# HuajianUP/Photo-SLAM

Hardware: AMD Instinct MI355X
Metric: train iters/s (render + L1/SSIM loss + backward + Adam), 2M Gaussians @1080p (higher is better)
Workload: dtype f32; 1 GPU; C3: Replica room0 @1080p shape; gaussians=2000000, width=1920, height=1080, sh_degree=3, parallelism=single GPU, raster_only=False, densify_interval=0, cull_empty_tiles=False, binning=depth-first, sh_adam_fused_into_backward=True, sh_adam_lazy_window=32, scene_index_order=random, geometry_adam_fused_into_backward=True, gaussians_after=2000000

## Files before the change

include/gsr.h:

```cpp
#ifndef GSR_H
#define GSR_H
#include <stddef.h>
#include <stdint.h>
#ifdef __cplusplus
extern "C" {
#endif

typedef enum gsr_status {
	GSR_OK = 0,
	GSR_ERR_INVALID_ARG = -1,
	GSR_ERR_ALLOC = -2,
	GSR_ERR_HIP = -3,
	GSR_ERR_UNSUPPORTED = -4
} gsr_status;

typedef char* (*gsr_alloc_fn)(void* ctx, size_t bytes);

#define GSR_SH_LAZY_WINDOW 32
typedef struct gsr_sh_adam_lazy {
	int* row_step;
	int window;
	double lr_past[GSR_SH_LAZY_WINDOW];
	double lr_tail_past[GSR_SH_LAZY_WINDOW];
} gsr_sh_adam_lazy;
// ... 120 lines not shown
	int packed_capacity_rows;
	const float* dL_ddepth;
	const float* dL_dalpha;
	float* dL_dviewmatrix;
	float* dL_dprojmatrix;
	float* dL_dcampos;
	char* pose_scratch;
	const gsr_geom_reg* geom_reg;
} gsr_backward_args;

int gsr_backward(const gsr_backward_args* args, void* stream);

int gsr_sh_adam_flush(int P, const gsr_sh_adam* adam, void* stream);

int gsr_sh_grad_from_views(int P, int D, int M, int n_views, const float* means3D, const float* campos,
                           long long campos_stride, const float* dL_dcolor_views, long long view_stride, float scale,
                           float* dL_dsh, void* stream);

int gsr_sh_adam_from_views(int P, int D, int M, int n_views, const float* means3D, const float* campos,
                           long long campos_stride, const float* dL_dcolor_views, long long view_stride, float scale,
                           float* shs, const gsr_sh_adam* sh_adam, void* stream);
size_t gsr_packed_view_words(int P, int capacity_rows);
int gsr_pack_view_plan(int P, const int* radii, uint32_t* message, void* scratch, void* stream);
size_t gsr_pack_scratch_bytes(int P);
int gsr_pack_color_view(int P, const float* dL_dcolor_view, const float* campos, int capacity_rows, uint32_t* message, void* scratch,
                        void* stream);
int gsr_sh_grad_from_packed_views(int P, int D, int M, int n_views, const float* means3D, const uint32_t* messages,
                                  long long msg_stride, float scale, float* dL_dsh, void* stream);
int gsr_sh_adam_from_packed_views(int P, int D, int M, int n_views, const float* means3D, const uint32_t* messages,
                                  long long msg_stride, float scale, float* shs, const gsr_sh_adam* sh_adam, void* stream);
int gsr_last_visible_count(void);
int gsr_last_forward_only(void);
long long gsr_depth_resort_count(void);
int gsr_binning_tile_first(int raw_params, int P, int width, int height);
int gsr_check_packed_views(int P, int n_views, const uint32_t* messages, long long msg_stride, int capacity_rows, void* stream);
int gsr_host_wait_stats(double* total_us, long long* calls, int reset);

int gsr_sh_adam_lazy_slice(int P, const gsr_sh_adam* adam, int ahead, void* stream);

int gsr_mark_visible(int P, const float* means3D, const float* viewmatrix, const float* projmatrix,
                     uint8_t* present, void* stream);

int gsr_knn_mean_dist2(int P, const float* points, float* meanDists,
                       gsr_alloc_fn scratchBuffer, void* scratch_ctx, void* stream);

size_t gsr_loss_scratch_bytes(int width, int height);
int gsr_l1_ssim_loss(const float* rendered, const float* gt, const float* mask, int width, int height,
                     float lambda_dssim, float* grad_rendered, float* loss, char* scratch, void* stream);

size_t gsr_loss_exposure_scratch_bytes(int width, int height);
int gsr_l1_ssim_loss_exposure(const float* rendered, const float* gt, const float* mask, int width, int height,
                              float lambda_dssim, const float* exposure, float* grad_rendered, float* grad_exposure,
                              float* loss, char* scratch, void* stream);
int gsr_apply_exposure(const float* image, const float* exposure, int width, int height, float* out, void* stream);

size_t gsr_depth_loss_scratch_bytes(int width, int height);
int gsr_depth_l1_loss(const float* depth, const float* gt_depth, int width, int height, float min_depth, float max_depth,
                      float weight, float* grad_depth, float* loss, char* scratch, void* stream);

int gsr_adam_step(float* param, const float* grad, float* exp_avg, float* exp_avg_sq, long long n, double lr,
                  double beta1, double beta2, double eps, int step, int period, int split, double lr_tail, void* stream);

typedef struct gsr_adam_multi_tensor {
	float* param;
	const float* grad;
	float* exp_avg;
// ... 77 lines not shown
```

photo-slam_amd/capi.py:

```python
import ctypes as C
import os

_HERE = os.path.dirname(os.path.abspath(__file__))
HIP_LIB_PATH = os.path.join(_HERE, "libgsr_hip.so")

ALLOC_FN = C.CFUNCTYPE(C.c_void_p, C.c_void_p, C.c_size_t)

GSR_OK = 0


class GsrError(RuntimeError):
    def __init__(self, lib, status, where):
        msg = lib.gsr_strerror(status).decode()
        hip = lib.gsr_last_hip_error_string().decode()
        super().__init__(f"{where}: {msg} (status {status})" + (f" [{hip}]" if status == -3 and hip else ""))
        self.status = status


class ForwardArgs(C.Structure):
    _fields_ = [("P", C.c_int), ("D", C.c_int), ("M", C.c_int), ("background", C.c_void_p),
                ("width", C.c_int), ("height", C.c_int), ("means3D", C.c_void_p), ("shs", C.c_void_p),
                ("colors_precomp", C.c_void_p), ("opacities", C.c_void_p), ("scales", C.c_void_p),
                ("scale_modifier", C.c_float), ("rotations", C.c_void_p), ("cov3D_precomp", C.c_void_p),
                ("viewmatrix", C.c_void_p), ("projmatrix", C.c_void_p), ("cam_pos", C.c_void_p),
# ... 79 lines not shown
                ("packed_view", C.c_void_p), ("packed_capacity_rows", C.c_int),
                ("dL_ddepth", C.c_void_p), ("dL_dalpha", C.c_void_p),
                ("dL_dviewmatrix", C.c_void_p), ("dL_dprojmatrix", C.c_void_p), ("dL_dcampos", C.c_void_p),
                ("pose_scratch", C.c_void_p), ("geom_reg", C.POINTER(GeomReg))]

class DensifySelectArgs(C.Structure):
    _fields_ = [("P", C.c_int), ("xyz_gradient_accum", C.c_void_p), ("denom", C.c_void_p), ("scaling", C.c_void_p),
                ("opacity", C.c_void_p), ("percent_dense", C.c_float), ("max_grad", C.c_float), ("min_opacity", C.c_float),
                ("extent", C.c_float), ("max_screen_size", C.c_int), ("prune_mask", C.c_void_p)]


class DensifyGatherArgs(C.Structure):
    _fields_ = [("P", C.c_int), ("n_new", C.c_int), ("n_keep", C.c_int), ("n_clone", C.c_int), ("n_child", C.c_int),
                ("n_split", C.c_int), ("features_row_floats", C.c_int),
                ("param_in", C.c_void_p * 5), ("exp_avg_in", C.c_void_p * 5), ("exp_avg_sq_in", C.c_void_p * 5),
                ("param_out", C.c_void_p * 5), ("exp_avg_out", C.c_void_p * 5), ("exp_avg_sq_out", C.c_void_p * 5),
                ("samples", C.c_void_p), ("stats_out", C.c_void_p * 3), ("exist_since_iter_in", C.c_void_p),
                ("exist_since_iter_out", C.c_void_p), ("morton_scratch", C.c_void_p)]


RAW_OPACITY, RAW_SCALING, RAW_ROTATION = 1, 2, 4
CULL_EMPTY_TILES, FORWARD_ONLY = 8, 128
ANTIALIAS = 256
CONTRIBUTION = 512


EXPORTED_SYMBOLS = [
    "gsr_forward", "gsr_backward", "gsr_mark_visible", "gsr_knn_mean_dist2", "gsr_geometry_bytes", "gsr_binning_bytes",
    "gsr_image_bytes", "gsr_knn_scratch_bytes", "gsr_sh_grad_from_views", "gsr_sh_adam_from_views", "gsr_sh_adam_flush", "gsr_sh_adam_lazy_slice", "gsr_adam_step_multi", "gsr_strerror", "gsr_last_hip_error", "gsr_last_hip_error_string",
    "gsr_backend", "gsr_profile_enable", "gsr_profile_stage_count", "gsr_profile_stage_name", "gsr_profile_read",
    "gsr_loss_scratch_bytes", "gsr_l1_ssim_loss", "gsr_adam_step", "gsr_densify_stats", "gsr_densify_scratch_bytes",
    "gsr_densify_select", "gsr_densify_gather", "gsr_transform_points", "gsr_scale_transform_points", "gsr_reproject_depth_pinhole",
    "gsr_neighborhood_depth_pinhole", "gsr_packed_view_words", "gsr_pack_scratch_bytes", "gsr_pack_color_view", "gsr_pack_view_plan",
    "gsr_sh_grad_from_packed_views", "gsr_sh_adam_from_packed_views", "gsr_last_visible_count", "gsr_check_packed_views", "gsr_depth_resort_count",
    "gsr_host_wait_stats", "gsr_binning_tile_first", "gsr_densify_morton_scratch_bytes",
    "gsr_binning_bytes_for", "gsr_image_bytes_for", "gsr_last_forward_only",
    "gsr_depth_loss_scratch_bytes", "gsr_depth_l1_loss", "gsr_pose_grad_scratch_bytes",
    "gsr_loss_exposure_scratch_bytes", "gsr_l1_ssim_loss_exposure", "gsr_apply_exposure",
    "gsr_geom_reg_scratch_bytes",
]

_libs = {}


def load(path=None):
    path = os.path.abspath(path or HIP_LIB_PATH)
    if path in _libs:
        return _libs[path]
    if not os.path.exists(path):
        raise FileNotFoundError(
            f"{path} not found: build the HIP extension first (python photo-slam_amd/build.py or "
            f"__graft_entry__.build()); there is no CPU fallback.")
    L = C.CDLL(path)
    vp, sz, i32, f32 = C.c_void_p, C.c_size_t, C.c_int, C.c_float
    L.gsr_forward.restype = i32
    L.gsr_forward.argtypes = [C.POINTER(ForwardArgs), ALLOC_FN, vp, ALLOC_FN, vp, ALLOC_FN, vp, vp, C.POINTER(i32)]
    L.gsr_backward.restype = i32
    L.gsr_backward.argtypes = [C.POINTER(BackwardArgs), vp]
    L.gsr_sh_grad_from_views.restype = i32
    L.gsr_sh_grad_from_views.argtypes = [i32, i32, i32, i32, vp, vp, C.c_longlong, vp, C.c_longlong, f32, vp, vp]
    L.gsr_sh_adam_from_views.restype = i32
    L.gsr_sh_adam_from_views.argtypes = [i32, i32, i32, i32, vp, vp, C.c_longlong, vp, C.c_longlong, f32, vp, C.POINTER(ShAdam), vp]
    L.gsr_sh_adam_flush.restype = i32
    L.gsr_sh_adam_flush.argtypes = [i32, C.POINTER(ShAdam), vp]
    L.gsr_sh_adam_lazy_slice.restype = i32
    L.gsr_sh_adam_lazy_slice.argtypes = [i32, C.POINTER(ShAdam), i32, vp]
    L.gsr_adam_step_multi.restype = i32
# ... 88 lines not shown
```

photo-slam_amd/csrc/gsr_api.hip:

```cpp
#include <atomic>
#include <chrono>
#include <cmath>
#include <vector>
#include "kernels.h"
#include "shrows.h"

#include <stdio.h>
#include <stdlib.h>
#include <string.h>

namespace gsr {

static thread_local int t_last_err = 0;
static thread_local char t_last_what[256] = {0};
void set_last_hip_error(int err, const char* what)
{
	t_last_err = err;
	snprintf(t_last_what, sizeof(t_last_what), "%s: %s", what ? what : "?", hipGetErrorString((hipError_t)err));
}

struct HostSync {
	uint32_t* pinned = nullptr;
	uint32_t* pinned_dev = nullptr;
	hipEvent_t ev = nullptr;
// ... 82 lines not shown
static bool lazy_slice_early(const gsr_sh_adam* o)
{
	static const int env = env_int("GSR_LAZY_SLICE_EARLY", -1);
	return env >= 0 ? env != 0 : !(o && o->lazy_slice_late);
}
static bool cov3D_stored()
{
	static const int env = env_int("GSR_COV3D_STORED", 0);
	return env != 0;
}
static bool emit_seeded()
{
	static const int env = env_int("GSR_EMIT_SEEDS", 1);
	return env != 0;
}
static int xcd_deal_mode(int tiles)
{
	static const int env = env_int("GSR_XCD_CHUNK", -1);
	if (env >= 0) return env;
	int c = 8;
	while (c > 1 && tiles < 8 * 16 * c) c >>= 1;
	return c;
}
static bool blend_bwd_half_tiles(int tiles)
{
	const char* e = getenv("GSR_BWD_HALF_TILES");
	if (e && *e) {
		static bool logged = false;
		if (!logged) fprintf(stderr, "[gsr] environment override GSR_BWD_HALF_TILES=%s\n", e);
		logged = true;
		return atoi(e) != 0;
	}
	return tiles >= 24 * 256;
}
static int depth_sort_wide()
{
	static const int on = env_int("GSR_DEPTH_SORT_9BIT", 1);
	static const int bits = env_int("GSR_DEPTH_SORT_BITS", 3 * RADIX_BITS_WIDE);
	if (!on) return 0;
	return (bits >= 1 && bits <= 27 && (div_up(bits, RADIX_BITS_WIDE) & 1)) ? bits : 3 * RADIX_BITS_WIDE;
}
static thread_local long long t_depth_resorts = 0;
static bool emit_hist()
{
	static const int env = env_int("GSR_EMIT_HIST", 1);
	return env != 0;
}
constexpr int TILE_FIRST_MAX_GAUSSIANS = 256 * 1024;
static bool binning_tile_first(int raw_params, int P, int tiles)
{
	static const int env = env_int("GSR_BINNING", -1);
	if (env >= 0) return env != 0;
	if (raw_params & GSR_BINNING_TILE_FIRST) return true;
	if (raw_params & GSR_BINNING_DEPTH_FIRST) return false;
	(void)tiles;
	return P <= TILE_FIRST_MAX_GAUSSIANS;
}
static int side_blocks(const gsr_sh_adam* o)
{
	static const int env = env_int("GSR_SH_ADAM_SIDE_BLOCKS", -1);
	return env >= 0 ? env : (o && o->side_blocks > 0 ? o->side_blocks : 256);
}

enum { ST_PREPROCESS = 0, ST_DEPTH_SORT, ST_OFFSET_SCAN, ST_EMIT, ST_TILE_SORT, ST_TILE_RANGES, ST_TILE_DEPTH_SORT, ST_BLEND_FWD,
       ST_GRAD_MEMSET, ST_BLEND_BWD, ST_PREPROCESS_BWD, ST_COUNT };
constexpr int ST_FWD_COUNT = ST_BLEND_FWD + 1;
// ... 424 lines not shown
	if (lazy && slice_early && (st = launch_lazy_slice()) != GSR_OK) return fail(st);
	PROF_BWD(0);
	if (R > 0 && !rows_path) GSR_HIP(hipMemsetAsync(bs.touched, 0, touched_clear_bytes((size_t)R), stream));
	PROF_BWD(1);
	if (R > 0) {
		BlendBwdParams bp;
		bp.ranges = im.ranges; bp.point_list = point_list; bp.rec = g.rec; bp.bg = a->background;
		bp.final_T = im.final_T; bp.n_contrib = im.n_contrib; bp.dL_dpix = a->dL_dpix;
		bp.partials = bs.partials;
		bp.touched = bs.touched;
		bp.contrib = bs.contrib; bp.contrib_stride = (size_t)R;
		bp.W = W; bp.H = H; bp.grid_x = grid_x; bp.tiles = tiles;
		bp.deal = make_tile_deal(tiles, grid_x, xcd_deal_mode(tiles));
		bp.half_tiles = blend_bwd_half_tiles(tiles) ? 1 : 0;
		bp.depth = reinterpret_cast<const float*>(g.depth_key);
		bp.dL_ddepth = a->dL_ddepth; bp.dL_dalpha = a->dL_dalpha;
		if ((st = launch_blend_bwd(bp, stream)) != GSR_OK) return fail(st);
	}
	PROF_BWD(2);
	if (lazy && !slice_early && (st = launch_lazy_slice()) != GSR_OK) return fail(st);

	PreprocessBwdParams pb;
	pb.P = P; pb.D = a->D; pb.M = a->M;
	pb.means3D = a->means3D; pb.radii = a->radii ? a->radii : g.radii; pb.shs = a->shs; pb.clamped = g.clamped;
	pb.scales = a->scales; pb.rotations = a->rotations; pb.scale_modifier = a->scale_modifier;
	pb.cov3D = a->cov3D_precomp;
	if (!pb.cov3D && cov3D_stored()) pb.cov3D = g.cov3D;
	pb.view = a->viewmatrix; pb.proj = a->projmatrix; pb.campos = a->campos;
	pb.focal_y = H / (2.0f * a->tan_fovy);
	pb.focal_x = W / (2.0f * a->tan_fovx);
	pb.tan_fovx = a->tan_fovx; pb.tan_fovy = a->tan_fovy;
	pb.tiles_touched = g.tiles_touched; pb.partials = R > 0 ? bs.partials : nullptr; pb.touched = R > 0 ? bs.touched : nullptr;
	pb.long_runs = g.long_runs; pb.long_counts = g.long_counts; pb.long_capacity = g.long_capacity;
	pb.half_w = 0.5f * (float)W; pb.half_h = 0.5f * (float)H;
	pb.rec = g.rec; pb.raw_params = a->raw_params;
	pb.dL_dmean2D = a->dL_dmean2D; pb.dL_dconic = a->dL_dconic; pb.dL_dopacity = a->dL_dopacity; pb.dL_dcolor = a->dL_dcolor;
	pb.dL_dmean3D = a->dL_dmean3D; pb.dL_dcov3D = a->dL_dcov3D; pb.dL_dsh = a->dL_dsh; pb.dL_dscale = a->dL_dscale;
	pb.dL_drot = a->dL_drot;
	pb.dL_dcolor_view = a->dL_dcolor_view;
	pb.packed_msg = a->dL_dcolor_view ? a->packed_view : nullptr;
	pb.packed_capacity = a->packed_capacity_rows;
	pb.stat_accum = a->stat_grad_accum; pb.stat_denom = a->stat_denom; pb.stat_max_radii = a->stat_max_radii;
	pb.adam_param = nullptr; pb.adam_exp_avg = nullptr; pb.adam_exp_avg_sq = nullptr;
	pb.adam = AdamScalars{};
	pb.adam_skip_culled = 0;
	pb.lazy_row_step = nullptr; pb.lazy_step = 0;
	pb.touched_clear = (R > 0 && rows_path) ? bs.touched : nullptr;
	pb.touched_clear_bytes = (uint32_t)touched_clear_bytes((size_t)R);
	if (a->sh_adam && !pre_slice) {
		const gsr_sh_adam& o = *a->sh_adam;
		pb.adam_param = o.param;
		pb.adam_exp_avg = o.exp_avg; pb.adam_exp_avg_sq = o.exp_avg_sq;
		pb.adam = adam_scalars(o.lr, o.lr_tail, o.beta1, o.beta2, o.eps, o.step);
		pb.adam_skip_culled = (side_busy || lazy) ? 1 : 0;
		if (lazy) { pb.lazy_row_step = la.row_step; pb.lazy_step = la.step; }
	}
	pb.geom = geom;
	pb.depth = (depth && R > 0) ? 1 : 0;
	pb.pose_scratch = pose ? reinterpret_cast<float*>(a->pose_scratch) : nullptr;
	pb.dL_dview = a->dL_dviewmatrix; pb.dL_dproj = a->dL_dprojmatrix; pb.dL_dcampos = a->dL_dcampos;
	pb.reg_on = reg ? 1 : 0;
	pb.reg_w_opacity = reg ? a->geom_reg->w_opacity : 0.f;
	pb.reg_w_scale = reg ? a->geom_reg->w_scale : 0.f;
	pb.reg_w_iso = reg ? a->geom_reg->w_isotropic : 0.f;
	pb.reg_slab = (reg && a->geom_reg->loss) ? reinterpret_cast<float*>(a->geom_reg->scratch) : nullptr;
	pb.reg_loss = reg ? a->geom_reg->loss : nullptr;
// ... 213 lines not shown
```

photo-slam_amd/csrc/kernels.h:

```cpp
#pragma once
#include "state.h"

#include <math.h>

namespace gsr {

struct AdamScalars {
	float step_size, step_size_tail, b1, b2, omb1, omb2, eps, inv_sqrt_bc2;
};
static inline AdamScalars adam_scalars(double lr, double lr_tail, double beta1, double beta2, double eps, int step)
{
	const double bc1 = 1.0 - pow(beta1, step), bc2 = 1.0 - pow(beta2, step);
	AdamScalars a;
	a.step_size = (float)(lr / bc1);
	a.step_size_tail = (float)(lr_tail / bc1);
	a.b1 = (float)beta1;
	a.b2 = (float)beta2;
	a.omb1 = (float)(1.0 - beta1);
	a.omb2 = (float)(1.0 - beta2);
	a.eps = (float)eps;
	a.inv_sqrt_bc2 = (float)(1.0 / sqrt(bc2));
	return a;
}

// ... 82 lines not shown

struct BlendBwdParams {
	const uint2* ranges;
	const uint32_t* point_list;
	const float4* rec;
	const float* bg;
	const float* final_T;
	const uint32_t* n_contrib;
	const float* dL_dpix;
	float* partials;
	uint8_t* touched;
	const uint8_t* contrib;
	size_t contrib_stride;
	int W, H, grid_x, tiles;
	TileDeal deal;
	int half_tiles;
	const float* depth;
	const float* dL_ddepth;
	const float* dL_dalpha;
};
int launch_blend_bwd(const BlendBwdParams& p, hipStream_t stream);

struct GeomAdamTensor {
	float* param;
	float* exp_avg;
	float* exp_avg_sq;
	AdamScalars s;
};
struct GeomAdam {
	int on;
	GeomAdamTensor xyz, opacity, scaling, rotation;
};

struct PreprocessBwdParams {
	int P, D, M;
	const float* means3D;
	const int* radii;
	const float* shs;
	const uint8_t* clamped;
	const float* scales;
	const float* rotations;
	float scale_modifier;
	const float* cov3D;
	const float* view;
	const float* proj;
	const float* campos;
	float focal_x, focal_y, tan_fovx, tan_fovy;
	const uint32_t* tiles_touched;
	float* partials;
	uint8_t* touched;
	const uint32_t* long_runs;
	const uint32_t* long_counts;
	uint32_t long_capacity;
	float half_w, half_h;
	const float4* rec;
	float* dL_dmean2D;
	float* dL_dconic;
	float* dL_dopacity;
	float* dL_dcolor;
	float* dL_dmean3D;
	float* dL_dcov3D;
	float* dL_dsh;
	float* dL_dcolor_view;
	float* dL_dscale;
	float* dL_drot;
	int raw_params;
	float* stat_accum;
	float* stat_denom;
	float* stat_max_radii;
	float* adam_param;
	float* adam_exp_avg;
	float* adam_exp_avg_sq;
	AdamScalars adam;
	int adam_skip_culled;
	int* lazy_row_step;
	int lazy_step;
	uint8_t* touched_clear;
	uint32_t touched_clear_bytes;
	GeomAdam geom;
	void* notify_stream;
	void* notify_event;
	uint32_t* packed_msg;
	int packed_capacity;
	int depth;
	float* pose_scratch;
	float* dL_dview;
	float* dL_dproj;
	float* dL_dcampos;
	int reg_on;
	float reg_w_opacity, reg_w_scale, reg_w_iso;
	float* reg_slab;
	float* reg_loss;
};
static inline size_t reg_slab_floats(int P) { return 3 * (((size_t)(P > 0 ? P : 0) + 127) / 128) + 4; }
int launch_reg_zero(float* loss, hipStream_t stream);
constexpr int POSE_VP = 24;
static inline size_t pose_slab_a_rows(int P) { return ((size_t)(P > 0 ? P : 0) + 127) / 128; }
static inline size_t pose_slab_b_rows(int P) { return ((size_t)(P > 0 ? P : 0) + 63) / 64; }
static inline size_t pose_slab_floats(int P) { return POSE_VP * pose_slab_a_rows(P) + 3 * pose_slab_b_rows(P) + 4; }
int launch_pose_zero(float* dL_dview, float* dL_dproj, float* dL_dcampos, hipStream_t stream);
int launch_preprocess_bwd(const PreprocessBwdParams& p, hipStream_t stream);
static inline bool sh_rows_path(const float* shs, int M, int D, bool factored, bool adam, const float* dL_dsh)
{
	return shs && 3 * M == 48 && (reinterpret_cast<uintptr_t>(shs) & 15) == 0 && D >= 0 && D <= 3 &&
	       (factored || adam || (dL_dsh && (reinterpret_cast<uintptr_t>(dL_dsh) & 15) == 0));
}
constexpr int PACK_HEADER = 8;
static inline size_t pack_groups(int P) { return ((size_t)P + 63) / 64; }
static inline size_t pack_prefix_words(int P) { return (pack_groups(P) + 3) & ~(size_t)3; }
static inline size_t pack_mask_words(int P) { return (2 * pack_groups(P) + 3) & ~(size_t)3; }
static inline size_t packed_view_words(int P, int capacity) { return PACK_HEADER + pack_prefix_words(P) + pack_mask_words(P) + 3 * (size_t)capacity + 4; }
int launch_pack_color_view(int P, const float* view, const float* campos, int capacity, uint32_t* msg, uint32_t* scratch, hipStream_t stream);
int launch_pack_view_plan(int P, const int* radii, uint32_t* msg, uint32_t* scratch, hipStream_t stream);
struct PackedViews {
	const uint32_t* msgs = nullptr;
	long long stride = 0;
};
struct RowAdam;
int launch_sh_grad_from_views(int P, int D, int M, int n_views, const float* means3D, const float* campos,
                              long long campos_stride, const float* dL_dcolor_views, long long view_stride, float scale,
                              float* dL_dsh, const RowAdam* adam, hipStream_t stream, const LazyAdam* lazy = nullptr,
                              PackedViews packed = PackedViews());

int launch_sh_adam_culled(int P, const int* radii, const RowAdam& adam, hipStream_t stream, int max_blocks);

// ... 49 lines not shown
```

photo-slam_amd/csrc/partials.h:

```cpp
#pragma once
#include "state.h"
#include "wave64.h"

namespace gsr {

template <int U, int N>
__device__ __forceinline__ void sum_slots_trip(const float4* src, unsigned long long& live, float (&a)[N])
{
	static_assert(N == 9 || N == 10, "nine sums, or ten with dL/dz");
	int idx[U];
	float4 x[U], y[U];
	float z[U], zd[U];
#pragma unroll
	for (int j = 0; j < U; j++) {
		idx[j] = __ffsll((long long)live) - 1;
		live &= live - 1ull;
	}
#pragma unroll
	for (int j = 0; j < U; j++) {
		x[j] = src[SLOT_F4 * (size_t)idx[j]];
		y[j] = src[SLOT_F4 * (size_t)idx[j] + 1];
		if constexpr (N == 10) {
			const float2 t = *reinterpret_cast<const float2*>(src + SLOT_F4 * (size_t)idx[j] + 2);
			z[j] = t.x;
			zd[j] = t.y;
		} else {
			z[j] = src[SLOT_F4 * (size_t)idx[j] + 2].x;
		}
	}
#pragma unroll
	for (int j = 0; j < U; j++) {
		a[0] += x[j].x; a[1] += x[j].y; a[2] += x[j].z; a[3] += x[j].w;
		a[4] += y[j].x; a[5] += y[j].y; a[6] += y[j].z; a[7] += y[j].w;
		a[8] += z[j];
		if constexpr (N == 10) a[9] += zd[j];
	}
}

__device__ __forceinline__ uint32_t squeeze_flags16(const uint8_t* p)
{
	uint4 f;
	__builtin_memcpy(&f, p, 16);
	return (((f.x * 0x01020408u) >> 24) & 0xFu) | ((((f.y * 0x01020408u) >> 24) & 0xFu) << 4) | ((((f.z * 0x01020408u) >> 24) & 0xFu) << 8) |
	       ((((f.w * 0x01020408u) >> 24) & 0xFu) << 12);
}

template <int N>
__device__ __forceinline__ void wave_sum_partial_runs(uint32_t cnt, uint32_t first, const float* __restrict__ partials,
                                                      const uint8_t* __restrict__ touched, float (&a)[N])
{
	const float4* part4 = reinterpret_cast<const float4*>(partials);
#pragma unroll
	for (int c = 0; c < N; c++) a[c] = 0.f;
	if (cnt != 0u && cnt <= LONG_RUN) {
		unsigned long long live = 0ull;
#pragma unroll
		for (int c = 0; c < 4; c++)
			if (16u * c < cnt) live |= (unsigned long long)squeeze_flags16(touched + first + 16 * c) << (16 * c);
		if (cnt < 64u) live &= (1ull << cnt) - 1ull;
		const float4* src = part4 + SLOT_F4 * (size_t)first;
		while (live & (live - 1ull)) sum_slots_trip<2>(src, live, a);
		while (live) sum_slots_trip<1>(src, live, a);
	}
	if (cnt > LONG_RUN && touched[first]) {
		const float4 x = part4[SLOT_F4 * (size_t)first], y = part4[SLOT_F4 * (size_t)first + 1];
		const float z = part4[SLOT_F4 * (size_t)first + 2].x;
		a[0] = x.x; a[1] = x.y; a[2] = x.z; a[3] = x.w;
		a[4] = y.x; a[5] = y.y; a[6] = y.z; a[7] = y.w;
		a[8] = z;
		if constexpr (N == 10) a[9] = part4[SLOT_F4 * (size_t)first + 2].y;
	}
}

template <bool DEPTH>
__device__ __forceinline__ void wave_sum_long_run(uint32_t first, uint32_t cnt, float* __restrict__ partials, uint8_t* __restrict__ touched)
{
	constexpr int N = DEPTH ? 10 : 9;
	const int l = lane_id();
	float4* part4 = reinterpret_cast<float4*>(partials);
	float v[N];
#pragma unroll
	for (int c = 0; c < N; c++) v[c] = 0.f;
	bool any = false;
	const uint32_t k = (cnt + 63u) >> 6;
	const uint32_t lo = (uint32_t)l * k, hi = min(cnt, lo + k);
	for (uint32_t g0 = lo; g0 < hi; g0 += 64u) {
		const uint32_t n = min(64u, hi - g0);
		unsigned long long live = 0ull;
#pragma unroll
		for (int c = 0; c < 4; c++)
			if (16u * c < n) live |= (unsigned long long)squeeze_flags16(touched + first + g0 + 16 * c) << (16 * c);
		if (n < 64u) live &= (1ull << n) - 1ull;
		any = any || live != 0ull;
		const float4* src = part4 + SLOT_F4 * (size_t)(first + g0);
		while (__popcll(live) >= 4) sum_slots_trip<4>(src, live, v);
		while (live & (live - 1ull)) sum_slots_trip<2>(src, live, v);
		while (live) sum_slots_trip<1>(src, live, v);
	}
	const bool some = wave_ballot(any) != 0ull;
	float v9 = 0.f;
	if constexpr (DEPTH) v9 = wave_sum_f32_lane63(v[9]);
	float (&v_nine)[9] = *reinterpret_cast<float (*)[9]>(&v[0]);
	wave_reduce9_f32(v_nine);
	if (l == 63) {
		part4[SLOT_F4 * (size_t)first] = make_float4(v[0], v[1], v[2], v[3]);
		part4[SLOT_F4 * (size_t)first + 1] = make_float4(v[4], v[5], v[6], v[7]);
		if constexpr (DEPTH) *reinterpret_cast<float2*>(part4 + SLOT_F4 * (size_t)first + 2) = make_float2(v[8], v9);
		else reinterpret_cast<float*>(part4 + SLOT_F4 * (size_t)first + 2)[0] = v[8];
		touched[first] = some ? 1 : 0;
	}
}

}
```

photo-slam_amd/csrc/preprocess_bwd.hip:

```cpp
#include "state.h"
#include "wave64.h"
#include <stdlib.h>
#include "kernels.h"
#include "shrows.h"
#include "partials.h"

namespace gsr {


constexpr int PRB_THREADS = 128;
constexpr int SHB_THREADS = 64;

template <int N>
struct GeomAdamRegs {
	float m[N], v[N], w[N];
};
template <int N>
__device__ __forceinline__ void geom_adam_load(const GeomAdamTensor& t, size_t idx, GeomAdamRegs<N>& r)
{
#pragma unroll
	for (int k = 0; k < N; k++) {
		const size_t i = (size_t)N * idx + k;
		r.m[k] = t.exp_avg[i];
		r.v[k] = t.exp_avg_sq[i];
		r.w[k] = t.param[i];
	}
}
template <int N>
__device__ __forceinline__ void geom_adam_finish(const GeomAdamTensor& t, size_t idx, const float (&g)[N], GeomAdamRegs<N>& r)
{
#pragma unroll
	for (int k = 0; k < N; k++) {
		r.m[k] = t.s.b1 * r.m[k] + t.s.omb1 * g[k];
		r.v[k] = t.s.b2 * r.v[k] + t.s.omb2 * g[k] * g[k];
		r.w[k] -= t.s.step_size * adam_ratio(r.m[k], r.v[k], t.s.inv_sqrt_bc2, t.s.eps);
	}
#pragma unroll
	for (int k = 0; k < N; k++) {
		const size_t i = (size_t)N * idx + k;
		t.exp_avg[i] = r.m[k];
		t.exp_avg_sq[i] = r.v[k];
		t.param[i] = r.w[k];
	}
// ... 155 lines not shown
	}
}

__device__ __forceinline__ void pack_view_row(const PreprocessBwdParams& p, int idx, bool vis, unsigned long long seen_mask, float v0, float v1,
                                              float v2)
{
	const size_t groups = ((size_t)p.P + 63) >> 6;
	const size_t prefix_words = (groups + 3) & ~(size_t)3, mask_words = (2 * groups + 3) & ~(size_t)3;
	uint32_t* msg = p.packed_msg;
	const size_t group = (size_t)idx >> 6;
	const uint32_t first = msg[PACK_HEADER + group];
	if (vis) {
		const uint32_t rank = first + (uint32_t)__popcll(seen_mask & lanemask_lt());
		if (rank < (uint32_t)p.packed_capacity) {
			float* rows = reinterpret_cast<float*>(msg + PACK_HEADER + prefix_words + mask_words);
			rows[3 * (size_t)rank] = v0;
			rows[3 * (size_t)rank + 1] = v1;
			rows[3 * (size_t)rank + 2] = v2;
		}
	}
	if (idx == p.P - 1) {
		const uint32_t K = first + (uint32_t)__popcll(seen_mask);
		msg[0] = K;
		msg[1] = (uint32_t)p.P;
		msg[2] = (uint32_t)p.packed_capacity;
		msg[3] = K > (uint32_t)p.packed_capacity ? 1u : 0u;
		msg[4] = __float_as_uint(p.campos[0]);
		msg[5] = __float_as_uint(p.campos[1]);
		msg[6] = __float_as_uint(p.campos[2]);
		msg[7] = 0u;
	}
}

template <bool ROWS_OK, bool PACKED = false, bool DEPTH = false, bool POSE = false, bool AA = false, bool REG = false>
__global__ void __launch_bounds__(PRB_THREADS)
preprocess_bwd_kernel(const PreprocessBwdParams p)
{
	__shared__ float s_pose[POSE ? PRB_THREADS / 64 : 1][POSE ? POSE_VP + 3 : 1];
	__shared__ float s_reg[REG ? PRB_THREADS / 64 : 1][REG ? 3 : 1];
	float reg_l[REG ? 3 : 1];
	if constexpr (REG) {
		reg_l[0] = reg_l[1] = reg_l[2] = 0.f;
	}
	float pose_v[POSE ? POSE_VP : 1];
	float pose_c[3] = {0.f, 0.f, 0.f};
	if constexpr (POSE) {
#pragma unroll
		for (int i = 0; i < POSE_VP; i++) pose_v[i] = 0.f;
	}

	const int idx = (int)(blockIdx.x * blockDim.x + threadIdx.x);
	const bool in_range = idx < p.P;
	const bool vis = in_range && (p.radii[idx] > 0);
	const int M3 = 3 * p.M;
	constexpr bool rows_ok = ROWS_OK;
	const unsigned long long seen_mask = PACKED ? wave_ballot(vis) : 0ull;

	float a[DEPTH ? 10 : 9];
	{
		const uint32_t cnt = (vis && p.partials) ? p.tiles_touched[idx] : 0u;
		const uint32_t first = cnt ? __float_as_uint(p.rec[3 * (size_t)idx + 2].w) : 0u;
		wave_sum_partial_runs(cnt, first, p.partials, p.touched, a);
	}
	float dL_dz = 0.f;
	if constexpr (DEPTH) dL_dz = a[9];
	float* out_sh = (p.dL_dsh && !p.dL_dcolor_view && !p.adam_exp_avg && in_range) ? p.dL_dsh + (size_t)idx * M3 : nullptr;

	if (!rows_ok && out_sh && !vis)
		for (int i = 0; i < M3; i++) out_sh[i] = 0.f;

	const float* V = p.view;
	const float* Pm = p.proj;
	float mx = 0.f, my = 0.f, mz = 0.f;
	float gmx = 0.f, gmy = 0.f, gmz = 0.f;
	float dcov[6] = {0.f, 0.f, 0.f, 0.f, 0.f, 0.f};
	float4 ga0 = make_float4(0.f, 0.f, 0.f, 0.f), ga1 = make_float4(0.f, 0.f, 0.f, 0.f);
	float g_opacity = 0.f;
	float aa_o = 0.f;

	if (vis) {
		mx = p.means3D[3 * (size_t)idx];
		my = p.means3D[3 * (size_t)idx + 1];
		mz = p.means3D[3 * (size_t)idx + 2];
		const float4 q0 = p.rec[3 * (size_t)idx];
		const float4 q1 = p.rec[3 * (size_t)idx + 1];
		const float A = q0.z, B = q0.w, C = q1.x, o = q1.y;
		ga0 = make_float4(a[0], a[1], a[2], -o * p.half_w * (a[3] * A + a[4] * B));
		ga1 = make_float4(-o * p.half_h * (a[4] * C + a[3] * B), -0.5f * o * a[5], -0.5f * o * a[6], -0.5f * o * a[7]);
		g_opacity = a[8];
		if constexpr (AA) {
			aa_o = o;
		} else {
			if (p.raw_params & GSR_RAW_OPACITY) g_opacity = g_opacity * o * (1.0f - o);
			if constexpr (REG) {
				g_opacity += (p.raw_params & GSR_RAW_OPACITY) ? p.reg_w_opacity * (o * (1.0f - o)) : p.reg_w_opacity;
				reg_l[0] = o;
// ... 340 lines not shown
				const float c = wave_sum_f32_lane63(pose_c[k]);
				if (l == 63) s_pose[w][POSE_VP + k] = c;
			}
		}
		__syncthreads();
		const int t = (int)threadIdx.x;
		if (t < (rows_ok ? POSE_VP : POSE_VP + 3)) {
			float sum = s_pose[0][t];
#pragma unroll
			for (int k = 1; k < PRB_THREADS / 64; k++) sum += s_pose[k][t];
			p.pose_scratch[(size_t)t * gridDim.x + blockIdx.x] = sum;
		}
	}
	if constexpr (REG) {
		if (p.reg_slab) {
			const int l = lane_id(), w = wave_id();
#pragma unroll
			for (int k = 0; k < 3; k++) {
				const float c = wave_sum_f32_lane63(reg_l[k]);
				if (l == 63) s_reg[w][k] = c;
			}
			__syncthreads();
			const int t = (int)threadIdx.x;
			if (t < 3) {
				float sum = s_reg[0][t];
#pragma unroll
				for (int k = 1; k < PRB_THREADS / 64; k++) sum += s_reg[k][t];
				p.reg_slab[(size_t)t * gridDim.x + blockIdx.x] = sum;
			}
		}
	}
}

__device__ __forceinline__ void sh_adam_culled_item(long long t, const int* __restrict__ radii, const RowAdam& a)
{
	const long long row = t / ROW_F4;
	if (radii[row] > 0) return;
	const int col = (int)(t - row * ROW_F4);
	const size_t i = (size_t)t;
	float4 pv = load_stream_f4(reinterpret_cast<const float4*>(a.param) + i);
	float4 mv = load_stream_f4(reinterpret_cast<const float4*>(a.exp_avg) + i);
	float4 vv = load_stream_f4(reinterpret_cast<const float4*>(a.exp_avg_sq) + i);
	float* pp = &pv.x; float* mp = &mv.x; float* vp = &vv.x;
	const float ss_first = col == 0 ? a.s.step_size : a.s.step_size_tail;
#pragma unroll
	for (int e = 0; e < 4; e++) {
		const float ss = e < 3 ? ss_first : a.s.step_size_tail;
		const float g = 0.f;
		mp[e] = a.s.b1 * mp[e] + a.s.omb1 * g;
		vp[e] = a.s.b2 * vp[e] + a.s.omb2 * g * g;
		pp[e] -= ss * adam_ratio(mp[e], vp[e], a.s.inv_sqrt_bc2, a.s.eps);
	}
	store_stream_f4(reinterpret_cast<float4*>(a.param) + i, pv);
	store_stream_f4(reinterpret_cast<float4*>(a.exp_avg) + i, mv);
	store_stream_f4(reinterpret_cast<float4*>(a.exp_avg_sq) + i, vv);
}

__global__ void __launch_bounds__(256)
sh_adam_culled_kernel(int P, const int* __restrict__ radii, const RowAdam a)
{
	const long long items = (long long)P * ROW_F4, stride = (long long)gridDim.x * 256;
	for (long long t = (long long)blockIdx.x * 256 + threadIdx.x; t < items; t += stride)
		sh_adam_culled_item(t, radii, a);
}

int launch_sh_adam_culled(int P, const int* radii, const RowAdam& adam, hipStream_t stream, int max_blocks)
// ... 32 lines not shown
			float4 mv = load_stream_f4(reinterpret_cast<const float4*>(a.exp_avg) + i);
			float4 vv = load_stream_f4(reinterpret_cast<const float4*>(a.exp_avg_sq) + i);
			lazy_zero_grad_steps(a.t, k_hi, k_lo, col, pv, mv, vv);
			store_stream_f4(reinterpret_cast<float4*>(a.param) + i, pv);
			store_stream_f4(reinterpret_cast<float4*>(a.exp_avg) + i, mv);
			store_stream_f4(reinterpret_cast<float4*>(a.exp_avg_sq) + i, vv);
		}
	}
	__syncthreads();
	if (mode == 3) {
		if (moved && col == 0) a.row_step[row] = a.step - 1;
	} else if (mine && col == 0) {
		a.row_step[row] = a.step;
	}
}

int launch_sh_adam_lazy(int P, const int* radii, const LazyAdam& a, hipStream_t stream, int mode)
{
	if (P <= 0) return GSR_OK;
	if (!a.row_step || a.window < 2 || a.window > LAZY_WINDOW_MAX || a.step < 1) return GSR_ERR_INVALID_ARG;
	if (mode == 3 && a.window < 3) return GSR_ERR_INVALID_ARG;
	if ((radii != nullptr) != (mode == 0)) return GSR_ERR_INVALID_ARG;
	if ((reinterpret_cast<uintptr_t>(a.param) | reinterpret_cast<uintptr_t>(a.exp_avg) | reinterpret_cast<uintptr_t>(a.exp_avg_sq)) & 15)
		return GSR_ERR_UNSUPPORTED;
	const int nb = div_up(P, LAZY_BLOCK_ROWS);
	const int period = mode == 3 ? a.window - 1 : a.window;
	const int phase = a.step % period;
	const int blocks = mode == 1 ? nb : (nb > phase ? div_up(nb - phase, period) : 0);
	if (blocks > 0) GSR_LAUNCH(sh_adam_lazy_kernel, blocks, LAZY_THREADS, stream, P, radii, a, mode);
	GSR_CHECK_LAUNCH();
	return GSR_OK;
}

constexpr int LRS_BLOCKS = 1024;
template <bool DEPTH>
__global__ void __launch_bounds__(256)
long_run_sums_kernel(const PreprocessBwdParams p)
{
	const uint32_t wave = (uint32_t)blockIdx.x * 4u + (uint32_t)wave_id(), waves = (uint32_t)gridDim.x * 4u;
	const uint32_t list = wave % (uint32_t)LONG_LISTS;
	const uint32_t n = p.long_counts[list * LONG_COUNT_STRIDE];
	for (uint32_t e = wave / (uint32_t)LONG_LISTS; e < n; e += waves / (uint32_t)LONG_LISTS) {
		const uint32_t g = p.long_runs[(size_t)list * p.long_capacity + e];
		const uint32_t cnt = p.tiles_touched[g];
		const uint32_t first = __float_as_uint(p.rec[3 * (size_t)g + 2].w);
		wave_sum_long_run<DEPTH>(first, cnt, p.partials, p.touched);
	}
}

constexpr int POSE_SUM_THREADS = 256;
__global__ void __launch_bounds__(POSE_SUM_THREADS)
pose_final_sum_kernel(const float* __restrict__ slab, unsigned n_a, unsigned n_b, float* __restrict__ dL_dview, float* __restrict__ dL_dproj,
                      float* __restrict__ dL_dcampos)
{
	__shared__ double s_sum[POSE_SUM_THREADS];
	const int comp = (int)blockIdx.x, t = (int)threadIdx.x;
	const bool vp = comp < POSE_VP;
	const unsigned n = vp ? n_a : n_b;
	const float* src = vp ? slab + (size_t)comp * n_a : slab + (size_t)POSE_VP * n_a + (size_t)(comp - POSE_VP) * n_b;
	double acc = 0.0;
	for (unsigned i = (unsigned)t; i < n; i += POSE_SUM_THREADS) acc += (double)src[i];
	s_sum[t] = acc;
	__syncthreads();
	for (int half = POSE_SUM_THREADS / 2; half > 0; half >>= 1) {
		if (t < half) s_sum[t] += s_sum[t + half];
		__syncthreads();
// ... 22 lines not shown
}

int launch_pose_zero(float* dL_dview, float* dL_dproj, float* dL_dcampos, hipStream_t stream)
{
	return launch_pose_final_sum(nullptr, 0u, 0u, dL_dview, dL_dproj, dL_dcampos, stream);
}

__global__ void __launch_bounds__(POSE_SUM_THREADS)
reg_final_sum_kernel(const float* __restrict__ slab, unsigned n, float w_opacity, float w_scale, float w_iso, float* __restrict__ loss)
{
	__shared__ double s_sum[POSE_SUM_THREADS];
	const int comp = (int)blockIdx.x, t = (int)threadIdx.x;
	const float* src = slab + (size_t)comp * n;
	double acc = 0.0;
	for (unsigned i = (unsigned)t; i < n; i += POSE_SUM_THREADS) acc += (double)src[i];
	s_sum[t] = acc;
	__syncthreads();
	for (int half = POSE_SUM_THREADS / 2; half > 0; half >>= 1) {
		if (t < half) s_sum[t] += s_sum[t + half];
		__syncthreads();
	}
	if (t == 0) loss[comp] = (float)((double)(comp == 0 ? w_opacity : (comp == 1 ? w_scale : w_iso)) * s_sum[0]);
}

int launch_reg_zero(float* loss, hipStream_t stream)
{
	GSR_LAUNCH(reg_final_sum_kernel, 3, POSE_SUM_THREADS, stream, (const float*)nullptr, 0u, 0.f, 0.f, 0.f, loss);
	GSR_CHECK_LAUNCH();
	return GSR_OK;
}

int launch_preprocess_bwd(const PreprocessBwdParams& p, hipStream_t stream)
{
	if (p.partials && p.depth) GSR_LAUNCH(long_run_sums_kernel<true>, LRS_BLOCKS, 256, stream, p);
	else if (p.partials) GSR_LAUNCH(long_run_sums_kernel<false>, LRS_BLOCKS, 256, stream, p);
	const bool factored = p.dL_dcolor_view != nullptr;
	const bool adam = p.adam_exp_avg != nullptr;
	const bool rows_ok = sh_rows_path(p.shs, p.M, p.D, factored, adam, p.dL_dsh);
	if (adam && (!rows_ok || factored || ((reinterpret_cast<uintptr_t>(p.adam_exp_avg) | reinterpret_cast<uintptr_t>(p.adam_exp_avg_sq)) & 15)))
		return GSR_ERR_UNSUPPORTED;
	if (p.geom.on && !(rows_ok && p.D >= 0 && p.D <= 3 && p.scales && p.rotations && p.dL_dmean3D))
		return GSR_ERR_UNSUPPORTED;
	const int grid = div_up(p.P, PRB_THREADS);
	const bool pose = p.pose_scratch != nullptr;
	unsigned pose_b_rows = 0u;
	if (pose && (factored || p.packed_msg)) return GSR_ERR_UNSUPPORTED;
	const bool aa = (p.raw_params & GSR_ANTIALIAS) != 0;
	const bool reg = p.reg_on != 0;
	if (reg && (pose || factored || p.packed_msg)) return GSR_ERR_UNSUPPORTED;
	if (reg && !p.scales && (p.reg_w_scale != 0.f || p.reg_w_iso != 0.f)) return GSR_ERR_INVALID_ARG;
#define GSR_PRB(RO, AAV)                                                                                                          \
	do {                                                                                                                          \
		if (reg && p.depth) GSR_LAUNCH((preprocess_bwd_kernel<RO, false, true, false, AAV, true>), grid, PRB_THREADS, stream, p);  \
		else if (reg) GSR_LAUNCH((preprocess_bwd_kernel<RO, false, false, false, AAV, true>), grid, PRB_THREADS, stream, p);      \
		else if (pose && p.depth) GSR_LAUNCH((preprocess_bwd_kernel<RO, false, true, true, AAV>), grid, PRB_THREADS, stream, p);       \
		else if (pose) GSR_LAUNCH((preprocess_bwd_kernel<RO, false, false, true, AAV>), grid, PRB_THREADS, stream, p);            \
		else if (p.packed_msg && p.depth) GSR_LAUNCH((preprocess_bwd_kernel<RO, true, true, false, AAV>), grid, PRB_THREADS, stream, p); \
		else if (p.packed_msg) GSR_LAUNCH((preprocess_bwd_kernel<RO, true, false, false, AAV>), grid, PRB_THREADS, stream, p);    \
		else if (p.depth) GSR_LAUNCH((preprocess_bwd_kernel<RO, false, true, false, AAV>), grid, PRB_THREADS, stream, p);         \
		else GSR_LAUNCH((preprocess_bwd_kernel<RO, false, false, false, AAV>), grid, PRB_THREADS, stream, p);                     \
	} while (0)
	if (rows_ok && p.D >= 0 && p.D <= 3) {
		if (aa) GSR_PRB(true, true);
		else GSR_PRB(true, false);
		GSR_CHECK_LAUNCH();
		if (p.notify_stream && p.notify_event) {
			GSR_HIP(hipEventRecord((hipEvent_t)p.notify_event, stream));
			GSR_HIP(hipStreamWaitEvent((hipStream_t)p.notify_stream, (hipEvent_t)p.notify_event, 0));
		}
		const int g = div_up(p.P, SHB_THREADS);
#define GSR_SHB(DEG)                                                                  \
	do {                                                                              \
		if (pose && DEG > 0 && adam)                                                  \
			GSR_LAUNCH((sh_bwd_rows_kernel<(DEG > 0 ? DEG : 1), 2, true>), g, SHB_THREADS, stream, p); \
		else if (pose && DEG > 0)                                                     \
			GSR_LAUNCH((sh_bwd_rows_kernel<(DEG > 0 ? DEG : 1), 0, true>), g, SHB_THREADS, stream, p); \
		else if (factored)                                                                 \
			GSR_LAUNCH((sh_bwd_rows_kernel<DEG, 1>), g, SHB_THREADS, stream, p);      \
		else if (adam)                                                                \
			GSR_LAUNCH((sh_bwd_rows_kernel<DEG, 2>), g, SHB_THREADS, stream, p);      \
		else                                                                          \
			GSR_LAUNCH((sh_bwd_rows_kernel<DEG, 0>), g, SHB_THREADS, stream, p);      \
	} while (0)
		if (p.D == 3)
			GSR_SHB(3);
		else if (p.D == 2)
			GSR_SHB(2);
		else if (p.D == 1)
			GSR_SHB(1);
		else
			GSR_SHB(0);
#undef GSR_SHB
		pose_b_rows = p.D > 0 ? (unsigned)g : 0u;
	} else {
		if (aa) GSR_PRB(false, true);
		else GSR_PRB(false, false);
// ... 269 lines not shown
		msg[4] = __float_as_uint(campos[0]);
		msg[5] = __float_as_uint(campos[1]);
		msg[6] = __float_as_uint(campos[2]);
		msg[7] = 0u;
	}
}

int launch_pack_color_view(int P, const float* view, const float* campos, int capacity, uint32_t* msg, uint32_t* scratch, hipStream_t stream)
{
	if (P <= 0) return GSR_OK;
	const int groups = (int)pack_groups(P), pw = (int)pack_prefix_words(P), mw = (int)pack_mask_words(P);
	uint32_t* prefix = msg + PACK_HEADER;
	GSR_LAUNCH(pack_mask_kernel, div_up(P, 256), 256, stream, P, view, prefix, prefix + pw);
	int st = launch_scan_u32(prefix, nullptr, prefix, groups, false, scratch, stream);
	if (st != GSR_OK) return st;
	GSR_LAUNCH(pack_rows_kernel, div_up(P, 256), 256, stream, P, view, campos, capacity, msg, pw, mw);
	GSR_CHECK_LAUNCH();
	return GSR_OK;
}

int launch_pack_view_plan(int P, const int* radii, uint32_t* msg, uint32_t* scratch, hipStream_t stream)
{
	if (P <= 0) return GSR_OK;
	const int groups = (int)pack_groups(P), pw = (int)pack_prefix_words(P);
	uint32_t* prefix = msg + PACK_HEADER;
	GSR_LAUNCH(pack_plan_kernel, div_up(P, 256), 256, stream, P, radii, prefix, prefix + pw);
	int st = launch_scan_u32(prefix, nullptr, prefix, groups, false, scratch, stream);
	if (st != GSR_OK) return st;
	GSR_CHECK_LAUNCH();
	return GSR_OK;
}

}
```

Measured before the change: 684.0 iters/s.

## Fold long-run partial sums into the preprocess backward launch via extra workgroups

```diff
diff --git a/include/gsr.h b/include/gsr.h
--- a/include/gsr.h
+++ b/include/gsr.h
@@ -176,6 +176,7 @@
 int gsr_last_visible_count(void);
 int gsr_last_forward_only(void);
 long long gsr_depth_resort_count(void);
+long long gsr_long_run_sum_launches(void);
 int gsr_binning_tile_first(int raw_params, int P, int width, int height);
 int gsr_check_packed_views(int P, int n_views, const uint32_t* messages, long long msg_stride, int capacity_rows, void* stream);
 int gsr_host_wait_stats(double* total_us, long long* calls, int reset);
diff --git a/photo-slam_amd/capi.py b/photo-slam_amd/capi.py
--- a/photo-slam_amd/capi.py
+++ b/photo-slam_amd/capi.py
@@ -135,7 +135,7 @@
     "gsr_loss_scratch_bytes", "gsr_l1_ssim_loss", "gsr_adam_step", "gsr_densify_stats", "gsr_densify_scratch_bytes",
     "gsr_densify_select", "gsr_densify_gather", "gsr_transform_points", "gsr_scale_transform_points", "gsr_reproject_depth_pinhole",
     "gsr_neighborhood_depth_pinhole", "gsr_packed_view_words", "gsr_pack_scratch_bytes", "gsr_pack_color_view", "gsr_pack_view_plan",
-    "gsr_sh_grad_from_packed_views", "gsr_sh_adam_from_packed_views", "gsr_last_visible_count", "gsr_check_packed_views", "gsr_depth_resort_count",
+    "gsr_sh_grad_from_packed_views", "gsr_sh_adam_from_packed_views", "gsr_last_visible_count", "gsr_check_packed_views", "gsr_depth_resort_count", "gsr_long_run_sum_launches",
     "gsr_host_wait_stats", "gsr_binning_tile_first", "gsr_densify_morton_scratch_bytes",
     "gsr_binning_bytes_for", "gsr_image_bytes_for", "gsr_last_forward_only",
     "gsr_depth_loss_scratch_bytes", "gsr_depth_l1_loss", "gsr_pose_grad_scratch_bytes",
diff --git a/photo-slam_amd/csrc/gsr_api.hip b/photo-slam_amd/csrc/gsr_api.hip
--- a/photo-slam_amd/csrc/gsr_api.hip
+++ b/photo-slam_amd/csrc/gsr_api.hip
@@ -138,6 +138,29 @@
 		return atoi(e) != 0;
 	}
 	return tiles >= 24 * 256;
+}
+static bool long_runs_inline()
+{
+	const char* e = getenv("GSR_LONG_RUNS_INLINE");
+	if (e && *e) {
+		static bool logged = false;
+		if (!logged) fprintf(stderr, "[gsr] environment override GSR_LONG_RUNS_INLINE=%s\n", e);
+		logged = true;
+		return atoi(e) != 0;
+	}
+	return true;
+}
+static int long_inline_wgs()
+{
+	const char* e = getenv("GSR_LONG_INLINE_WGS");
+	if (e && *e) {
+		static bool logged = false;
+		if (!logged) fprintf(stderr, "[gsr] environment override GSR_LONG_INLINE_WGS=%s\n", e);
+		logged = true;
+		const int n = atoi(e);
+		if (n >= 1 && n <= 65536) return div_up(n, LONG_WGS_STEP) * LONG_WGS_STEP;
+	}
+	return LONG_WGS_DEFAULT;
 }
 static int depth_sort_wide()
 {
@@ -628,6 +651,7 @@
 	pb.tan_fovx = a->tan_fovx; pb.tan_fovy = a->tan_fovy;
 	pb.tiles_touched = g.tiles_touched; pb.partials = R > 0 ? bs.partials : nullptr; pb.touched = R > 0 ? bs.touched : nullptr;
 	pb.long_runs = g.long_runs; pb.long_counts = g.long_counts; pb.long_capacity = g.long_capacity;
+	pb.long_inline = long_runs_inline() ? 1 : 0; pb.long_wgs = long_inline_wgs();
 	pb.half_w = 0.5f * (float)W; pb.half_h = 0.5f * (float)H;
 	pb.rec = g.rec; pb.raw_params = a->raw_params;
 	pb.dL_dmean2D = a->dL_dmean2D; pb.dL_dconic = a->dL_dconic; pb.dL_dopacity = a->dL_dopacity; pb.dL_dcolor = a->dL_dcolor;
diff --git a/photo-slam_amd/csrc/kernels.h b/photo-slam_amd/csrc/kernels.h
--- a/photo-slam_amd/csrc/kernels.h
+++ b/photo-slam_amd/csrc/kernels.h
@@ -138,6 +138,7 @@
 	GeomAdamTensor xyz, opacity, scaling, rotation;
 };
 
+constexpr int LONG_WGS_STEP = 32, LONG_WGS_DEFAULT = 2048;
 struct PreprocessBwdParams {
 	int P, D, M;
 	const float* means3D;
@@ -197,6 +198,8 @@
 	float reg_w_opacity, reg_w_scale, reg_w_iso;
 	float* reg_slab;
 	float* reg_loss;
+	int long_inline;
+	int long_wgs;
 };
 static inline size_t reg_slab_floats(int P) { return 3 * (((size_t)(P > 0 ? P : 0) + 127) / 128) + 4; }
 int launch_reg_zero(float* loss, hipStream_t stream);
diff --git a/photo-slam_amd/csrc/partials.h b/photo-slam_amd/csrc/partials.h
--- a/photo-slam_amd/csrc/partials.h
+++ b/photo-slam_amd/csrc/partials.h
@@ -45,7 +45,7 @@
 	       ((((f.w * 0x01020408u) >> 24) & 0xFu) << 12);
 }
 
-template <int N>
+template <int N, bool FOLDED = true>
 __device__ __forceinline__ void wave_sum_partial_runs(uint32_t cnt, uint32_t first, const float* __restrict__ partials,
                                                       const uint8_t* __restrict__ touched, float (&a)[N])
 {
@@ -62,7 +62,7 @@
 		while (live & (live - 1ull)) sum_slots_trip<2>(src, live, a);
 		while (live) sum_slots_trip<1>(src, live, a);
 	}
-	if (cnt > LONG_RUN && touched[first]) {
+	if (FOLDED && cnt > LONG_RUN && touched[first]) {
 		const float4 x = part4[SLOT_F4 * (size_t)first], y = part4[SLOT_F4 * (size_t)first + 1];
 		const float z = part4[SLOT_F4 * (size_t)first + 2].x;
 		a[0] = x.x; a[1] = x.y; a[2] = x.z; a[3] = x.w;
@@ -72,13 +72,14 @@
 	}
 }
 
-template <bool DEPTH>
-__device__ __forceinline__ void wave_sum_long_run(uint32_t first, uint32_t cnt, float* __restrict__ partials, uint8_t* __restrict__ touched)
+constexpr int LONG_INLINE_TRIP = 2;
+template <bool DEPTH, int MAX_TRIP = 4>
+__device__ __forceinline__ bool wave_sum_long_run_regs(uint32_t first, uint32_t cnt, const float* __restrict__ partials,
+                                                       const uint8_t* __restrict__ touched, float (&v)[DEPTH ? 10 : 9])
 {
 	constexpr int N = DEPTH ? 10 : 9;
 	const int l = lane_id();
-	float4* part4 = reinterpret_cast<float4*>(partials);
-	float v[N];
+	const float4* part4 = reinterpret_cast<const float4*>(partials);
 #pragma unroll
 	for (int c = 0; c < N; c++) v[c] = 0.f;
 	bool any = false;
@@ -93,7 +94,8 @@
 		if (n < 64u) live &= (1ull << n) - 1ull;
 		any = any || live != 0ull;
 		const float4* src = part4 + SLOT_F4 * (size_t)(first + g0);
-		while (__popcll(live) >= 4) sum_slots_trip<4>(src, live, v);
+		if constexpr (MAX_TRIP >= 4)
+			while (__popcll(live) >= 4) sum_slots_trip<4>(src, live, v);
 		while (live & (live - 1ull)) sum_slots_trip<2>(src, live, v);
 		while (live) sum_slots_trip<1>(src, live, v);
 	}
@@ -102,10 +104,20 @@
 	if constexpr (DEPTH) v9 = wave_sum_f32_lane63(v[9]);
 	float (&v_nine)[9] = *reinterpret_cast<float (*)[9]>(&v[0]);
 	wave_reduce9_f32(v_nine);
-	if (l == 63) {
+	if constexpr (DEPTH) v[9] = v9;
+	return some;
+}
+
+template <bool DEPTH>
+__device__ __forceinline__ void wave_sum_long_run(uint32_t first, uint32_t cnt, float* __restrict__ partials, uint8_t* __restrict__ touched)
+{
+	float v[DEPTH ? 10 : 9];
+	const bool some = wave_sum_long_run_regs<DEPTH>(first, cnt, partials, touched, v);
+	float4* part4 = reinterpret_cast<float4*>(partials);
+	if (lane_id() == 63) {
 		part4[SLOT_F4 * (size_t)first] = make_float4(v[0], v[1], v[2], v[3]);
 		part4[SLOT_F4 * (size_t)first + 1] = make_float4(v[4], v[5], v[6], v[7]);
-		if constexpr (DEPTH) *reinterpret_cast<float2*>(part4 + SLOT_F4 * (size_t)first + 2) = make_float2(v[8], v9);
+		if constexpr (DEPTH) *reinterpret_cast<float2*>(part4 + SLOT_F4 * (size_t)first + 2) = make_float2(v[8], v[9]);
 		else reinterpret_cast<float*>(part4 + SLOT_F4 * (size_t)first + 2)[0] = v[8];
 		touched[first] = some ? 1 : 0;
 	}
diff --git a/photo-slam_amd/csrc/preprocess_bwd.hip b/photo-slam_amd/csrc/preprocess_bwd.hip
--- a/photo-slam_amd/csrc/preprocess_bwd.hip
+++ b/photo-slam_amd/csrc/preprocess_bwd.hip
@@ -9,6 +9,7 @@
 
 
 constexpr int PRB_THREADS = 128;
+static_assert(LONG_WGS_STEP * (PRB_THREADS / 64) == LONG_LISTS, "the extra workgroups' waves: a multiple of the sub-lists (kernels.h)");
 constexpr int SHB_THREADS = 64;
 
 template <int N>
@@ -230,9 +231,9 @@
 	}
 }
 
-template <bool ROWS_OK, bool PACKED = false, bool DEPTH = false, bool POSE = false, bool AA = false, bool REG = false>
-__global__ void __launch_bounds__(PRB_THREADS)
-preprocess_bwd_kernel(const PreprocessBwdParams p)
+template <bool ROWS_OK, bool PACKED, bool DEPTH, bool POSE, bool AA, bool REG>
+__device__ __forceinline__ void preprocess_bwd_row(const PreprocessBwdParams& p, const int idx, const bool in_range, const bool vis,
+                                                   const float (&a)[DEPTH ? 10 : 9])
 {
 	__shared__ float s_pose[POSE ? PRB_THREADS / 64 : 1][POSE ? POSE_VP + 3 : 1];
 	__shared__ float s_reg[REG ? PRB_THREADS / 64 : 1][REG ? 3 : 1];
@@ -247,19 +248,10 @@
 		for (int i = 0; i < POSE_VP; i++) pose_v[i] = 0.f;
 	}
 
-	const int idx = (int)(blockIdx.x * blockDim.x + threadIdx.x);
-	const bool in_range = idx < p.P;
-	const bool vis = in_range && (p.radii[idx] > 0);
 	const int M3 = 3 * p.M;
 	constexpr bool rows_ok = ROWS_OK;
 	const unsigned long long seen_mask = PACKED ? wave_ballot(vis) : 0ull;
 
-	float a[DEPTH ? 10 : 9];
-	{
-		const uint32_t cnt = (vis && p.partials) ? p.tiles_touched[idx] : 0u;
-		const uint32_t first = cnt ? __float_as_uint(p.rec[3 * (size_t)idx + 2].w) : 0u;
-		wave_sum_partial_runs(cnt, first, p.partials, p.touched, a);
-	}
 	float dL_dz = 0.f;
 	if constexpr (DEPTH) dL_dz = a[9];
 	float* out_sh = (p.dL_dsh && !p.dL_dcolor_view && !p.adam_exp_avg && in_range) ? p.dL_dsh + (size_t)idx * M3 : nullptr;
@@ -666,6 +658,54 @@
 	}
 }
 
+template <bool ROWS_OK, bool PACKED = false, bool DEPTH = false, bool POSE = false, bool AA = false, bool REG = false, bool LONG_INLINE = false>
+__global__ void __launch_bounds__(PRB_THREADS) GSR_WAVES_PER_EU((LONG_INLINE && !AA) ? 8 : 1, 8)
+preprocess_bwd_kernel(const PreprocessBwdParams p)
+{
+	static_assert(!LONG_INLINE || (ROWS_OK && !PACKED && !POSE && !REG), "the in-launch long runs: plain training kernels only");
+	bool extra = false;
+	uint32_t lr_list = 0u, lr_e = 0u, lr_n = 0u, lr_step = 1u;
+	if constexpr (LONG_INLINE) {
+		extra = blockIdx.x < (unsigned)p.long_wgs;
+		if (extra) {
+			const uint32_t wave = wave_uniform_u32((uint32_t)blockIdx.x * (PRB_THREADS / 64) + (uint32_t)wave_id());
+			lr_list = wave % (uint32_t)LONG_LISTS;
+			lr_e = wave / (uint32_t)LONG_LISTS;
+			lr_step = (uint32_t)p.long_wgs * (PRB_THREADS / 64) / (uint32_t)LONG_LISTS;
+			lr_n = p.long_counts[lr_list * LONG_COUNT_STRIDE];
+		}
+	}
+	for (;;) {
+		float a[DEPTH ? 10 : 9];
+		int idx;
+		bool in_range, vis;
+		if (LONG_INLINE && extra) {
+			if (lr_e >= lr_n) return;
+			idx = (int)p.long_runs[(size_t)lr_list * p.long_capacity + lr_e];
+			lr_e += lr_step;
+			const uint32_t cnt = p.tiles_touched[idx];
+			const uint32_t first = __float_as_uint(p.rec[3 * (size_t)idx + 2].w);
+			wave_sum_long_run_regs<DEPTH, LONG_INLINE_TRIP>(first, cnt, p.partials, p.touched, a);
+			in_range = vis = lane_id() == 63;
+		} else {
+			idx = (int)((blockIdx.x - (LONG_INLINE ? (unsigned)p.long_wgs : 0u)) * blockDim.x + threadIdx.x);
+			in_range = idx < p.P;
+			vis = in_range && (p.radii[idx] > 0);
+			uint32_t cnt = (vis && p.partials) ? p.tiles_touched[idx] : 0u;
+			if constexpr (LONG_INLINE) {
+				if (cnt > LONG_RUN) {
+					in_range = vis = false;
+					cnt = 0u;
+				}
+			}
+			const uint32_t first = cnt ? __float_as_uint(p.rec[3 * (size_t)idx + 2].w) : 0u;
+			wave_sum_partial_runs<(DEPTH ? 10 : 9), !LONG_INLINE>(cnt, first, p.partials, p.touched, a);
+		}
+		preprocess_bwd_row<ROWS_OK, PACKED, DEPTH, POSE, AA, REG>(p, idx, in_range, vis, a);
+		if (!(LONG_INLINE && extra)) return;
+	}
+}
+
 __device__ __forceinline__ void sh_adam_culled_item(long long t, const int* __restrict__ radii, const RowAdam& a)
 {
 	const long long row = t / ROW_F4;
@@ -764,6 +804,7 @@
 	return GSR_OK;
 }
 
+static thread_local long long t_long_run_sum_launches = 0;
 constexpr int LRS_BLOCKS = 1024;
 template <bool DEPTH>
 __global__ void __launch_bounds__(256)
@@ -852,11 +893,16 @@
 
 int launch_preprocess_bwd(const PreprocessBwdParams& p, hipStream_t stream)
 {
-	if (p.partials && p.depth) GSR_LAUNCH(long_run_sums_kernel<true>, LRS_BLOCKS, 256, stream, p);
-	else if (p.partials) GSR_LAUNCH(long_run_sums_kernel<false>, LRS_BLOCKS, 256, stream, p);
 	const bool factored = p.dL_dcolor_view != nullptr;
 	const bool adam = p.adam_exp_avg != nullptr;
 	const bool rows_ok = sh_rows_path(p.shs, p.M, p.D, factored, adam, p.dL_dsh);
+	const bool long_inline = p.long_inline && p.partials && rows_ok && !factored && !p.packed_msg && !p.pose_scratch && !p.reg_on;
+	if (long_inline && (p.long_wgs < LONG_WGS_STEP || p.long_wgs % LONG_WGS_STEP != 0)) return GSR_ERR_INVALID_ARG;
+	if (p.partials && !long_inline) {
+		t_long_run_sum_launches++;
+		if (p.depth) GSR_LAUNCH(long_run_sums_kernel<true>, LRS_BLOCKS, 256, stream, p);
+		else GSR_LAUNCH(long_run_sums_kernel<false>, LRS_BLOCKS, 256, stream, p);
+	}
 	if (adam && (!rows_ok || factored || ((reinterpret_cast<uintptr_t>(p.adam_exp_avg) | reinterpret_cast<uintptr_t>(p.adam_exp_avg_sq)) & 15)))
 		return GSR_ERR_UNSUPPORTED;
 	if (p.geom.on && !(rows_ok && p.D >= 0 && p.D <= 3 && p.scales && p.rotations && p.dL_dmean3D))
@@ -881,7 +927,13 @@
 		else GSR_LAUNCH((preprocess_bwd_kernel<RO, false, false, false, AAV>), grid, PRB_THREADS, stream, p);                     \
 	} while (0)
 	if (rows_ok && p.D >= 0 && p.D <= 3) {
-		if (aa) GSR_PRB(true, true);
+		if (long_inline) {
+			const int grid_li = grid + p.long_wgs;
+			if (aa && p.depth) GSR_LAUNCH((preprocess_bwd_kernel<true, false, true, false, true, false, true>), grid_li, PRB_THREADS, stream, p);
+			else if (aa) GSR_LAUNCH((preprocess_bwd_kernel<true, false, false, false, true, false, true>), grid_li, PRB_THREADS, stream, p);
+			else if (p.depth) GSR_LAUNCH((preprocess_bwd_kernel<true, false, true, false, false, false, true>), grid_li, PRB_THREADS, stream, p);
+			else GSR_LAUNCH((preprocess_bwd_kernel<true, false, false, false, false, false, true>), grid_li, PRB_THREADS, stream, p);
+		} else if (aa) GSR_PRB(true, true);
 		else GSR_PRB(true, false);
 		GSR_CHECK_LAUNCH();
 		if (p.notify_stream && p.notify_event) {
@@ -1217,3 +1269,5 @@
 }
 
 }
+
+long long gsr_long_run_sum_launches(void) { return gsr::t_long_run_sum_launches; }
```

Measured after the change: 687.0 iters/s (median of 6 runs). No clear change (+0.4%).
